# cruiseresearchgroup/ViLCo

Hardware: AMD Instinct MI355X
Metric: clips/sec (fwd+bwd) MQ transformer T=2304 C=2304 (higher is better)
Workload: dtype fp16 MFMA on 2-part splits of power-of-two scaled fp32 operands (22 significant bits, 3 MFMAs per product), fp32 accumulate: fp32-equivalent; weight-gradient products with contraction length >= 2048 use the leading fp16 parts only (11-bit operands, 1 MFMA; <= 3.5e-4 of the 3-MFMA gradients at this c; 1 GPU; MQ ViLCo backbone config P: T=2304 Cin=2304 D=1024 H=16 arch(2,2,5) XLNet layer text L=77x768 22 classes, train mode with the reference's dropout 0.1 / droppath 0.1 / XLNet dropout 0.1 (mq_vilco.yaml, xlnet_config_1024.json); clips_per_gpu=2, global_batch=2, parallelism=dp1

## Files before the change

vilco_amd/csrc/attn.hip:

```cpp
#include <type_traits>
#include "common.h"
#define VILCO_TU "attn"
#include "pack.h"

typedef __attribute__((ext_vector_type(4))) __bf16 bf16x4;
typedef __attribute__((ext_vector_type(4))) _Float16 f16x4;

namespace {

constexpr int ATT_THREADS = 256;

template <int W>
__device__ __forceinline__ int swzc(int row, int chunk) {
  if (W == 32) return chunk ^ ((4 - ((row >> 2) & 3)) & 3);
  if (W == 64) return chunk ^ ((row >> 1) & 7);
  if (W == 160) return (chunk & ~3) | ((chunk & 3) ^ ((4 - ((row >> 2) & 3)) & 3));
  return chunk ^ (row & 15);
}
template <int W>
__device__ __forceinline__ int toff(int row, int chunk) { return row * W + (swzc<W>(row, chunk) << 3); }

template <int NP>
__device__ __forceinline__ void split8(const float (&v)[8], bf16x8 (&part)[3]) {
#pragma unroll
// ... 349 lines not shown
      for (int q = 0; q < NP; ++q) pb[q] = frag<BKV>(myP + q * 16 * BKV, fb64, 0, ks);
#pragma unroll
      for (int di = 0; di < HDP / 16; ++di) {
        bf16x8 va[3];
#pragma unroll
        for (int q = 0; q < NP; ++q) va[q] = frag<BKV>(sVt + q * HDP * BKV, fb64, di * 16, ks);
        oacc[di] = mfma_parts<NP, F16>(va, pb, oacc[di]);
      }
    }
  }

  if (qi < a.Tq) {
    const float inv = (l_run > 0.f ? 1.f / l_run : 0.f) * (F16 ? P_INV * sc.iv : 1.f) * a.drop_inv_keep;
    float* og = a.o + ((long)b * a.Tq + qi) * ld + h * a.hd;
#pragma unroll
    for (int di = 0; di < HDP / 16; ++di) {
      const int d = di * 16 + (lane >> 4) * 4;
      if (d + 4 <= a.hd) {
        *reinterpret_cast<float4*>(og + d) = make_float4(oacc[di][0] * inv, oacc[di][1] * inv, oacc[di][2] * inv, oacc[di][3] * inv);
      } else {
#pragma unroll
        for (int r = 0; r < 4; ++r) if (d + r < a.hd) og[d + r] = oacc[di][r] * inv;
      }
    }
    if (a.lse && (lane >> 4) == 0) a.lse[(long)bh * a.Tq + qi] = m_run + logf(l_run);
  }
}

__device__ __forceinline__ f32x4 mfma3h(const bf16x8 (&a)[2], const bf16x8 (&b)[2], f32x4 c) {
  const f16x8 a0 = __builtin_bit_cast(f16x8, a[0]), a1 = __builtin_bit_cast(f16x8, a[1]);
  const f16x8 b0 = __builtin_bit_cast(f16x8, b[0]), b1 = __builtin_bit_cast(f16x8, b[1]);
  c = __builtin_amdgcn_mfma_f32_16x16x32_f16(a1, b0, c, 0, 0, 0);
  c = __builtin_amdgcn_mfma_f32_16x16x32_f16(a0, b1, c, 0, 0, 0);
  return __builtin_amdgcn_mfma_f32_16x16x32_f16(a0, b0, c, 0, 0, 0);
}

constexpr int F64_Q = 128;

__device__ __forceinline__ void block_amax_out(float m, float* out, float* smem_f) {
  m = wave_max(m);
  __syncthreads();
  if ((threadIdx.x & 63) == 0) smem_f[threadIdx.x >> 6] = m;
  __syncthreads();
  if (threadIdx.x == 0)
    out[(blockIdx.z * gridDim.y + blockIdx.y) * gridDim.x + blockIdx.x] = fmaxf(fmaxf(smem_f[0], smem_f[1]), fmaxf(smem_f[2], smem_f[3]));
}
constexpr int RS64 = 80;
constexpr int PL64 = 64 * RS64;

__device__ __forceinline__ bf16x8 tr_frag64(const __bf16* p) {
  typedef short s16x4 __attribute__((ext_vector_type(4)));
  const s16x4 lo = __builtin_amdgcn_ds_read_tr16_b64_v4i16((__attribute__((address_space(3))) s16x4*)(p));
  const s16x4 hi = __builtin_amdgcn_ds_read_tr16_b64_v4i16((__attribute__((address_space(3))) s16x4*)(p + 16 * RS64));
  return __builtin_bit_cast(bf16x8, __builtin_shufflevector(lo, hi, 0, 1, 2, 3, 4, 5, 6, 7));
}


#ifdef VILCO_LAB_ATTN
__device__ unsigned long long vilco_lab_attn_stamps[64 * 8];
#define ASTAMP(i)                                                                                             \
  do {                                                                                                         \
    if (stamp_on && stamp_t < 64) {                                                                            \
      const unsigned long long c_ = __builtin_amdgcn_s_memtime();                                              \
      asm volatile("s_waitcnt lgkmcnt(0)" ::: "memory");                                                       \
      if (lane == 0) vilco_lab_attn_stamps[stamp_t * 8 + (i)] = c_;                                            \
    }                                                                                                          \
  } while (0)
#else
#define ASTAMP(i) do {} while (0)
#endif

template <int NR>
__device__ __forceinline__ void xl_dma_rows(const float* bias, int ld, int Tq, int q_first, unsigned voff, unsigned lds0) {
#pragma unroll
  for (int r = 0; r < NR; ++r) {
    int qi = q_first + r;
    qi = qi < Tq ? qi : Tq - 1;
    const float* row = bias + ((long)qi * (ld - 1) + Tq);
    asm volatile("s_mov_b32 m0, %0\n\ts_nop 0\n\tglobal_load_lds_dword %1, %2" ::"s"(lds0 + (unsigned)r * 272u), "v"(voff), "s"(row) : "memory");
  }
}
__device__ __forceinline__ unsigned lds_addr_of(const void* p) {
  return (unsigned)(uintptr_t)(__attribute__((address_space(3))) const void*)p;
}

template <bool XL>
__global__ __launch_bounds__(ATT_THREADS, 2) void attn_fwd64_kernel(AttnArgs a) {
  if (a.drop_thresh) a.drop_seed = vilco_step_seed(a.drop_seed, a.seed_word);
  constexpr int HDP = 64, BKV = 64;
  extern __shared__ __attribute__((aligned(16))) unsigned char smem_raw[];
  __bf16* sK = reinterpret_cast<__bf16*>(smem_raw);
  __bf16* sV = sK + 2 * PL64;

  const int tid = threadIdx.x, lane = tid & 63, wave = tid >> 6;
  const int h = blockIdx.y, b = blockIdx.z;
  const int bh = b * a.H + h;
  const int q0 = blockIdx.x * F64_Q + wave * 32;
  const int len = a.mode == 2 ? a.Tk : a.kv_len[b];
  const int kend = XL ? a.Tk : (len < a.Tk ? len : a.Tk);
  const int ntiles = (kend + BKV - 1) / BKV;
  const AttnScales sc = *a.sc;
  const int bias_ld = a.Tq + a.Tk;
  const float* bias = XL ? a.bias + ((long)bh * a.Tq) * bias_ld : nullptr;
  constexpr int RSBF = 68;
  float* sBias = reinterpret_cast<float*>(sV + 2 * PL64) + wave * 32 * RSBF;
  const int q0s = __builtin_amdgcn_readfirstlane(q0);
  const unsigned sbias_lds = XL ? (unsigned)__builtin_amdgcn_readfirstlane((int)lds_addr_of(sBias)) : 0u;
  [[maybe_unused]] auto bias_dma = [&](int k0, int g) {
    const int j = k0 + lane;
    xl_dma_rows<16>(bias, bias_ld, a.Tq, q0s + 16 * g, 4u * (unsigned)(j < a.Tk ? j : a.Tk - 1), sbias_lds + (unsigned)g * 16u * 272u);
  };
  const float c2 = a.scale * sc.iq * sc.ik * 1.44269504088896340736f;
  const __bf16* kbase = a.kn.p + (long)bh * a.kn.batch_stride;
  const __bf16* vbase = a.vn.p + (long)bh * a.vn.batch_stride;
  const int g4 = lane >> 4;
  const int fbn = (lane & 15) * RS64 + g4 * 8;
  const int fbt = (4 * g4 + ((lane & 15) >> 2)) * RS64 + 4 * (lane & 3);

  QFrag<HDP, 2> qf[2];
#pragma unroll
  for (int g = 0; g < 2; ++g) load_qfrag<HDP, 2>(qf[g], a.qn, a.qn.p + (long)bh * a.qn.batch_stride, q0 + 16 * g, lane);

  f32x4 oacc[2][4];
#pragma unroll
  for (int g = 0; g < 2; ++g)
#pragma unroll
    for (int i = 0; i < 4; ++i) oacc[g][i] = f32x4{0.f, 0.f, 0.f, 0.f};
  float m_run[2] = {-INFINITY, -INFINITY}, l_run[2] = {0.f, 0.f};
  [[maybe_unused]] uint32_t rkey[2] = {0u, 0u};
  if constexpr (XL) {
    if (a.drop_thresh) { rkey[0] = drop_row(a, bh, q0 + (lane & 15)); rkey[1] = drop_row(a, bh, q0 + 16 + (lane & 15)); }
  }

  bf16x8 stK[2][2], stV[2][2];
  const int srow = tid >> 3, sc8 = tid & 7;
  auto gload = [&](int k0) {
#pragma unroll
    for (int i = 0; i < 2; ++i) {
      int kr = k0 + srow + 32 * i;
      kr = kr < a.kn.rows ? kr : a.kn.rows - 1;
#pragma unroll
      for (int q = 0; q < 2; ++q) {
        stK[q][i] = *reinterpret_cast<const bf16x8*>(kbase + q * a.kn.part_stride + (long)kr * HDP + sc8 * 8);
        stV[q][i] = *reinterpret_cast<const bf16x8*>(vbase + q * a.vn.part_stride + (long)kr * HDP + sc8 * 8);
      }
    }
  };
  auto lstore = [&]() {
#pragma unroll
    for (int i = 0; i < 2; ++i) {
      const int o = (srow + 32 * i) * RS64 + sc8 * 8;
#pragma unroll
      for (int q = 0; q < 2; ++q) {
        *reinterpret_cast<bf16x8*>(sK + q * PL64 + o) = stK[q][i];
        *reinterpret_cast<bf16x8*>(sV + q * PL64 + o) = stV[q][i];
      }
    }
  };

  typedef float f32x2 __attribute__((ext_vector_type(2)));
  typedef _Float16 f16x2 __attribute__((ext_vector_type(2)));
  typedef uint32_t u32x4 __attribute__((ext_vector_type(4)));
  const f32x2 c2v = {c2, c2};
#ifdef VILCO_LAB_ATTN
  const bool stamp_on = blockIdx.x == 0 && blockIdx.y == 0 && blockIdx.z == 0 && wave == 0;
#endif
// ... 68 lines not shown
      }
      float mx = fmaxf(fmaxf(s[g][0][0], s[g][0][1]), fmaxf(s[g][0][2], s[g][0][3]));
#pragma unroll
      for (int mi = 1; mi < 4; ++mi) mx = fmaxf(mx, fmaxf(fmaxf(s[g][mi][0], s[g][mi][1]), fmaxf(s[g][mi][2], s[g][mi][3])));
      mx = quad16_max(mx);
      const float m_new = fmaxf(m_run[g], mx);
      const bool dead = XL && m_new == -INFINITY;
      const float alpha = dead ? 1.f : __builtin_amdgcn_exp2f(m_run[g] - m_new);
      const float off = dead ? 0.f : 15.f - m_new;
      const f32x2 offv = {off, off};
      f32x2 psum = {0.f, 0.f};
#pragma unroll
      for (int ks = 0; ks < 2; ++ks) {
        u32x4 h0, h1;
#pragma unroll
        for (int e = 0; e < 8; e += 2) {
          const f32x2 sv = {s[g][2 * ks + (e >> 2)][e & 3], s[g][2 * ks + (e >> 2)][(e & 3) + 1]};
          const f32x2 arg = sv + offv;
          f32x2 p = {__builtin_amdgcn_exp2f(arg[0]), __builtin_amdgcn_exp2f(arg[1])};
          psum += p;
          if constexpr (XL) {
            if (a.drop_thresh) {
              const uint32_t jw = jw0 + (uint32_t)((2 * ks + (e >> 2)) * 16 + (e & 3)) * VILCO_ATTN_DROP_W;
              p[0] = vilco_attn_drop_keep_w(rkey[g], jw, a.drop_thresh) ? p[0] : 0.f;
              p[1] = vilco_attn_drop_keep_w(rkey[g], jw + VILCO_ATTN_DROP_W, a.drop_thresh) ? p[1] : 0.f;
            }
          }
          const f16x2 hp = {(_Float16)p[0], (_Float16)p[1]};
          const uint32_t hpu = __builtin_bit_cast(uint32_t, hp);
          uint32_t lo;
          asm("v_fma_mixlo_f16 %0, %1, -1.0, %2 op_sel_hi:[1,0,0]" : "=v"(lo) : "v"(hpu), "v"(p[0]));
          asm("v_fma_mixhi_f16 %0, %1, -1.0, %2 op_sel:[1,0,0] op_sel_hi:[1,0,0]" : "+v"(lo) : "v"(hpu), "v"(p[1]));
          h0[e >> 1] = hpu;
          h1[e >> 1] = lo;
        }
        pb[g][ks][0] = __builtin_bit_cast(bf16x8, h0);
        pb[g][ks][1] = __builtin_bit_cast(bf16x8, h1);
      }
      l_run[g] = l_run[g] * alpha + (psum[0] + psum[1]);
      m_run[g] = m_new;
      if (__any(alpha != 1.f)) {
#pragma unroll
        for (int i = 0; i < 4; ++i) { oacc[g][i][0] *= alpha; oacc[g][i][1] *= alpha; oacc[g][i][2] *= alpha; oacc[g][i][3] *= alpha; }
      }
      if constexpr (XL) {
        if (more) {
          asm volatile("s_waitcnt lgkmcnt(0)" ::: "memory");
          bias_dma(k0 + BKV, g);
        }
      }
    }
    ASTAMP(3);
    bf16x8 vf[2][2];
#pragma unroll
    for (int q = 0; q < 2; ++q) vf[0][q] = tr_frag64(sV + q * PL64 + fbt);
#pragma unroll
    for (int st = 0; st < 8; ++st) {
      const int ks = st >> 2, di = st & 3;
      if (st + 1 < 8) {
#pragma unroll
        for (int q = 0; q < 2; ++q) vf[(st + 1) & 1][q] = tr_frag64(sV + q * PL64 + fbt + ((st + 1) >> 2) * 32 * RS64 + ((st + 1) & 3) * 16);
      }
      const f16x8 v0h = __builtin_bit_cast(f16x8, vf[st & 1][0]), v1h = __builtin_bit_cast(f16x8, vf[st & 1][1]);
      const f16x8 a0 = __builtin_bit_cast(f16x8, pb[0][ks][0]), a1 = __builtin_bit_cast(f16x8, pb[0][ks][1]);
      const f16x8 b0 = __builtin_bit_cast(f16x8, pb[1][ks][0]), b1 = __builtin_bit_cast(f16x8, pb[1][ks][1]);
      f32x4 c0 = oacc[0][di], c1 = oacc[1][di];
      c0 = __builtin_amdgcn_mfma_f32_16x16x32_f16(v1h, a0, c0, 0, 0, 0);
      c1 = __builtin_amdgcn_mfma_f32_16x16x32_f16(v1h, b0, c1, 0, 0, 0);
      c0 = __builtin_amdgcn_mfma_f32_16x16x32_f16(v0h, a1, c0, 0, 0, 0);
      c1 = __builtin_amdgcn_mfma_f32_16x16x32_f16(v0h, b1, c1, 0, 0, 0);
      c0 = __builtin_amdgcn_mfma_f32_16x16x32_f16(v0h, a0, c0, 0, 0, 0);
      c1 = __builtin_amdgcn_mfma_f32_16x16x32_f16(v0h, b0, c1, 0, 0, 0);
      oacc[0][di] = c0; oacc[1][di] = c1;
    }
    ASTAMP(5);
  };

  if (ntiles > 0) gload(0);
  if constexpr (XL) { if (ntiles > 0) { bias_dma(0, 0); bias_dma(0, 1); } }
  const int nfull = (XL ? (len < a.Tk ? len : a.Tk) : kend) / BKV;
  for (int t = 0; t < nfull; ++t) tile(t, t + 1 < ntiles, std::false_type{});
  for (int t = nfull; t < ntiles; ++t) tile(t, t + 1 < ntiles, std::true_type{});

  typedef _Float16 h4o __attribute__((ext_vector_type(4)));
  const float so = a.op0 ? sc.sv * a.o_scale_mul : 0.f;
  float am = 0.f;
#pragma unroll
  for (int g = 0; g < 2; ++g) {
    float l = l_run[g];
    l = quad16_sum(l);
    const int qi = q0 + 16 * g + (lane & 15);
    if (qi < a.Tq) {
      const float inv = (l > 0.f ? 1.f / l : 0.f) * sc.iv * (XL ? a.drop_inv_keep : 1.f);
      float* og = a.o + ((long)b * a.Tq + qi) * a.C + h * HDP;
#pragma unroll
      for (int di = 0; di < 4; ++di) {
        const float4 v = make_float4(oacc[g][di][0] * inv, oacc[g][di][1] * inv, oacc[g][di][2] * inv, oacc[g][di][3] * inv);
        *reinterpret_cast<float4*>(og + di * 16 + g4 * 4) = v;
        am = fmaxf(fmaxf(am, fmaxf(fabsf(v.x), fabsf(v.y))), fmaxf(fabsf(v.z), fabsf(v.w)));
        if (a.op0) {
          const float xs[4] = {v.x * so, v.y * so, v.z * so, v.w * so};
          h4o h0, h1;
#pragma unroll
          for (int e = 0; e < 4; ++e) { h0[e] = (_Float16)xs[e]; h1[e] = (_Float16)(xs[e] - (float)h0[e]); }
          const long po = ((long)b * a.Tq + qi) * a.C + h * HDP + di * 16 + g4 * 4;
          *reinterpret_cast<h4o*>(a.op0 + po) = h0;
          *reinterpret_cast<h4o*>(a.op0 + a.o_plane_stride + po) = h1;
        }
      }
      if (a.lse && g4 == 0) a.lse[(long)bh * a.Tq + qi] = 0.69314718055994530942f * (m_run[g] + __builtin_amdgcn_logf(l) - 15.f);
    }
  }
  if (a.op0) {
    if ((blockIdx.x | blockIdx.y | blockIdx.z) == 0 && tid == 0) { a.o_inv_scale[0] = sc.iv / a.o_scale_mul; a.o_inv_scale[1] = so; }
    if (blockIdx.x == gridDim.x - 1 && b == a.B - 1) {
      const long rows = (long)a.B * a.Tq;
      const h4o hz = {(_Float16)0.f, (_Float16)0.f, (_Float16)0.f, (_Float16)0.f};
      for (long i = tid; i < (a.o_rows32 - rows) * 16; i += ATT_THREADS) {
        const long po = (rows + i / 16) * a.C + h * HDP + (i % 16) * 4;
        *reinterpret_cast<h4o*>(a.op0 + po) = hz;
        *reinterpret_cast<h4o*>(a.op0 + a.o_plane_stride + po) = hz;
      }
    }
  }
  if (a.am_o) block_amax_out(am, a.am_o, reinterpret_cast<float*>(smem_raw));
}

__global__ __launch_bounds__(ATT_THREADS, 2) void xl_scores64_kernel(AttnArgs a) {
  constexpr int HDP = 64;
  extern __shared__ __attribute__((aligned(16))) unsigned char smem_raw[];
  __bf16* sK = reinterpret_cast<__bf16*>(smem_raw);
  const int tid = threadIdx.x, lane = tid & 63, wave = tid >> 6;
  const int h = blockIdx.y, b = blockIdx.z;
  const int bh = b * a.H + h;
  const int T = a.Tq, P = 2 * a.Tq;
  const int Q0 = blockIdx.x * F64_Q, q0 = Q0 + wave * 32;
  const AttnScales sc = *a.sc;
  const float unscale = sc.iq * sc.ik;
  const __bf16* kbase = a.kn.p + (long)(a.mode ? bh : h) * a.kn.batch_stride;
  const int g4 = lane >> 4;
  const int fbn = (lane & 15) * RS64 + g4 * 8;

  QFrag<HDP, 2> qf[2];
#pragma unroll
  for (int g = 0; g < 2; ++g) load_qfrag<HDP, 2>(qf[g], a.qn, a.qn.p + (long)bh * a.qn.batch_stride, q0 + 16 * g, lane);

  bf16x8 stK[2][2];
  const int srow = tid >> 3, sc8 = tid & 7;
  auto gload = [&](int p0) {
#pragma unroll
    for (int i = 0; i < 2; ++i) {
      int kr = p0 + srow + 32 * i;
      kr = kr < a.kn.rows ? kr : a.kn.rows - 1;
#pragma unroll
      for (int q = 0; q < 2; ++q) stK[q][i] = *reinterpret_cast<const bf16x8*>(kbase + q * a.kn.part_stride + (long)kr * HDP + sc8 * 8);
    }
  };
  auto lstore = [&]() {
#pragma unroll
    for (int i = 0; i < 2; ++i) {
      const int o = (srow + 32 * i) * RS64 + sc8 * 8;
#pragma unroll
      for (int q = 0; q < 2; ++q) *reinterpret_cast<bf16x8*>(sK + q * PL64 + o) = stK[q][i];
    }
  };
  const int qlast = (Q0 + F64_Q - 1 < T ? Q0 + F64_Q - 1 : T - 1);
  const int t_lo = (T - qlast) / 64, t_hi = (P - Q0 + 63) / 64;
  float* orow[2];
  int irow[2];
#pragma unroll
  for (int g = 0; g < 2; ++g) {
    irow[g] = q0 + 16 * g + (lane & 15);
    orow[g] = a.o + ((long)bh * T + (irow[g] < T ? irow[g] : T - 1)) * P;
  }
  if (t_lo < t_hi) gload(t_lo * 64);
  for (int t = t_lo; t < t_hi; ++t) {
    const int p0 = t * 64;
    __syncthreads();
    lstore();
    __syncthreads();
    if (t + 1 < t_hi) gload(p0 + 64);
    if (p0 + 63 < T - (q0 + 31) || p0 >= P - q0) continue;
    f32x4 s[2][4];
    bf16x8 kf[2][2];
#pragma unroll
    for (int q = 0; q < 2; ++q) kf[0][q] = *reinterpret_cast<const bf16x8*>(sK + q * PL64 + fbn);
#pragma unroll
    for (int st = 0; st < 8; ++st) {
      const int mi = st >> 1, ks = st & 1;
      if (st + 1 < 8) {
#pragma unroll
        for (int q = 0; q < 2; ++q)
          kf[(st + 1) & 1][q] = *reinterpret_cast<const bf16x8*>(sK + q * PL64 + fbn + ((st + 1) >> 1) * 16 * RS64 + ((st + 1) & 1) * 32);
      }
      const f16x8 k0h = __builtin_bit_cast(f16x8, kf[st & 1][0]), k1h = __builtin_bit_cast(f16x8, kf[st & 1][1]);
      const f16x8 a0 = __builtin_bit_cast(f16x8, qf[0].f[ks][0]), a1 = __builtin_bit_cast(f16x8, qf[0].f[ks][1]);
      const f16x8 b0 = __builtin_bit_cast(f16x8, qf[1].f[ks][0]), b1 = __builtin_bit_cast(f16x8, qf[1].f[ks][1]);
      f32x4 c0 = ks ? s[0][mi] : f32x4{0.f, 0.f, 0.f, 0.f}, c1 = ks ? s[1][mi] : f32x4{0.f, 0.f, 0.f, 0.f};
      c0 = __builtin_amdgcn_mfma_f32_16x16x32_f16(k1h, a0, c0, 0, 0, 0);
      c1 = __builtin_amdgcn_mfma_f32_16x16x32_f16(k1h, b0, c1, 0, 0, 0);
      c0 = __builtin_amdgcn_mfma_f32_16x16x32_f16(k0h, a1, c0, 0, 0, 0);
      c1 = __builtin_amdgcn_mfma_f32_16x16x32_f16(k0h, b1, c1, 0, 0, 0);
      c0 = __builtin_amdgcn_mfma_f32_16x16x32_f16(k0h, a0, c0, 0, 0, 0);
      c1 = __builtin_amdgcn_mfma_f32_16x16x32_f16(k0h, b0, c1, 0, 0, 0);
      s[0][mi] = c0; s[1][mi] = c1;
    }
#pragma unroll
    for (int g = 0; g < 2; ++g) {
// ... 900 lines not shown
      const int off = toff<BQ>(ncol + (lane & 15), mq * 2 + (lane >> 5)) + ((lane >> 4) & 1) * 4;
#pragma unroll
      for (int q = 0; q < NP; ++q) {
        *reinterpret_cast<bf16x4*>(sPt + q * BKV * BQ + off) = pp[q];
        *reinterpret_cast<bf16x4*>(sdSt + q * BKV * BQ + off) = dd[q];
      }
    }
    __syncthreads();

    bf16x8 pb[3], sb[3];
#pragma unroll
    for (int q = 0; q < NP; ++q) {
      pb[q] = frag<BQ>(sPt + q * BKV * BQ, fb32, wave * 16, 0);
      sb[q] = frag<BQ>(sdSt + q * BKV * BQ, fb32, wave * 16, 0);
    }
#pragma unroll
    for (int di = 0; di < HDP / 16; ++di) {
      bf16x8 oa[3], qa[3];
#pragma unroll
      for (int q = 0; q < NP; ++q) {
        oa[q] = frag<BQ>(sdOt + q * HDP * BQ, fb32, di * 16, 0);
        qa[q] = frag<BQ>(sQt + q * HDP * BQ, fb32, di * 16, 0);
      }
      dvacc[di] = mfma_parts<NP, F16>(oa, pb, dvacc[di]);
      dkacc[di] = mfma_parts<NP, F16>(qa, sb, dkacc[di]);
    }
  }

  const int key = k0 + wave * 16 + (lane & 15);
  if (key < a.Tk) {
    float* gk = a.dk + ((long)b * a.Tk + key) * ld + h * a.hd;
    float* gv = a.dv + ((long)b * a.Tk + key) * ld + h * a.hd;
#pragma unroll
    for (int di = 0; di < HDP / 16; ++di) {
      const int d = di * 16 + (lane >> 4) * 4;
#pragma unroll
      for (int r = 0; r < 4; ++r) {
        if (d + r < a.hd) {
          gk[d + r] = dkacc[di][r] * (a.scale * ds_unscale * sc.iq);
          gv[d + r] = dvacc[di][r] * ((F16 ? P_INV * sc.ido : 1.f) * a.drop_inv_keep);
        }
      }
    }
  }
}

template <int HDP, int NP>
size_t fwd_lds() { return (size_t)NP * (64 * HDP + HDP * 64 + 4 * 16 * 64) * sizeof(__bf16); }
template <int HDP, int NP>
size_t dq_lds() { return (size_t)NP * (3 * 64 * HDP + 4 * 16 * 64) * sizeof(__bf16); }
template <int HDP, int NP>
size_t dkdv_lds() {
  return (size_t)NP * ((HDP > 128 ? 64 * HDP : 2 * 64 * HDP) + 4 * 32 * HDP + 2 * 64 * 32) * sizeof(__bf16);
}

template <typename K>
void set_lds(K kernel, size_t bytes) {
  hipFuncSetAttribute(reinterpret_cast<const void*>(kernel), hipFuncAttributeMaxDynamicSharedMemorySize, (int)bytes);
  (void)hipGetLastError();
}

bool fwd64_enabled();
inline bool fast64(const AttnArgs& a, int precision) {
  return precision == 3 && a.hd == 64 && !a.bias && !a.dbias && (a.mode == 0 || a.mode == 2) && !a.drop_thresh && fwd64_enabled();
}
bool xl64_enabled();
inline bool fast64_xl_fwd(const AttnArgs& a, int precision) {
  return precision == 3 && a.hd == 64 && a.bias && a.mode == 3 && a.Tq == a.Tk && fwd64_enabled() && xl64_enabled();
}
bool xl64_enabled() { static const bool on = [] { const char* e = getenv("VILCO_ATTN_XL_FAST"); return !(e && e[0] == '0'); }(); return on; }
bool fwd64_enabled() { static const bool on = [] { const char* e = getenv("VILCO_ATTN_FAST"); return !(e && e[0] == '0'); }(); return on; }

template <int HDP, int NP, bool F16 = false>
int launch_fwd(const AttnArgs& a, hipStream_t s) {
  if constexpr (HDP == 64 && NP == 2 && F16) {
    if (fast64(a, 3)) {
      size_t lds = 2 * 2 * PL64 * sizeof(__bf16);
#ifdef VILCO_LAB_ATTN
      if (const char* e = getenv("VILCO_LAB_ATTN_LDS")) {
        lds = (size_t)atoi(e);
        hipFuncSetAttribute(reinterpret_cast<const void*>(&attn_fwd64_kernel<false>), hipFuncAttributeMaxDynamicSharedMemorySize, (int)lds);
      }
#endif
      hipLaunchKernelGGL(attn_fwd64_kernel<false>, dim3((a.Tq + F64_Q - 1) / F64_Q, a.H, a.B), dim3(ATT_THREADS), lds, s, a);
      return vilco_launch_status();
    }
    if (fast64_xl_fwd(a, 3)) {
      const size_t lds = 2 * 2 * PL64 * sizeof(__bf16) + 4 * 32 * 68 * sizeof(float);
      static const bool oncexl = [] { set_lds(&attn_fwd64_kernel<true>, 2 * 2 * PL64 * sizeof(__bf16) + 4 * 32 * 68 * sizeof(float)); return true; }();
      (void)oncexl;
      hipLaunchKernelGGL(attn_fwd64_kernel<true>, dim3((a.Tq + F64_Q - 1) / F64_Q, a.H, a.B), dim3(ATT_THREADS), lds, s, a);
      return vilco_launch_status();
    }
  }
  static const bool once = [] {
    set_lds(&attn_fwd_kernel<HDP, NP, F16, false>, fwd_lds<HDP, NP>());
    set_lds(&attn_fwd_kernel<HDP, NP, F16, true>, fwd_lds<HDP, NP>());
    return true;
  }();
  (void)once;
  dim3 grid((a.Tq + 63) / 64, a.H, a.B);
  const size_t lds = fwd_lds<HDP, NP>();
  if (a.drop_thresh) hipLaunchKernelGGL((attn_fwd_kernel<HDP, NP, F16, true>), grid, dim3(ATT_THREADS), lds, s, a);
  else hipLaunchKernelGGL((attn_fwd_kernel<HDP, NP, F16, false>), grid, dim3(ATT_THREADS), lds, s, a);
  return vilco_launch_status();
}

struct ForkCtx { hipStream_t s2; hipEvent_t e0, e1; };

inline ForkCtx* attn_fork(hipStream_t s) {
  static const bool enabled = [] { const char* e = getenv("VILCO_ATTN_FORK"); return e && e[0] == '1'; }();
  if (!enabled) return nullptr;
  hipStreamCaptureStatus st = hipStreamCaptureStatusNone;
  if (hipStreamIsCapturing(s, &st) != hipSuccess) return nullptr;
  static ForkCtx ctx;
  static int state = 0;
  if (st != hipStreamCaptureStatusActive) {
    if (state == 0)
      state = (hipStreamCreateWithFlags(&ctx.s2, hipStreamNonBlocking) == hipSuccess &&
               hipEventCreateWithFlags(&ctx.e0, hipEventDisableTiming) == hipSuccess &&
               hipEventCreateWithFlags(&ctx.e1, hipEventDisableTiming) == hipSuccess) ? 1 : -1;
    return nullptr;
  }
  return state == 1 ? &ctx : nullptr;
}

template <int HDP, int NP, bool F16 = false>
int launch_bwd(const AttnArgs& a, hipStream_t s) {
  static const bool once = [] {
    set_lds(&attn_bwd_dq_kernel<HDP, NP, F16, false>, dq_lds<HDP, NP>());
    set_lds(&attn_bwd_dq_kernel<HDP, NP, F16, true>, dq_lds<HDP, NP>());
    set_lds(&attn_bwd_dkdv_kernel<HDP, NP, F16, false, false>, dkdv_lds<HDP, NP>());
    set_lds(&attn_bwd_dkdv_kernel<HDP, NP, F16, true, false>, dkdv_lds<HDP, NP>());
    set_lds(&attn_bwd_dkdv_kernel<HDP, NP, F16, false, true>, dkdv_lds<HDP, NP>());
    set_lds(&attn_bwd_dkdv_kernel<HDP, NP, F16, true, true>, dkdv_lds<HDP, NP>());
    return true;
  }();
  (void)once;
  dim3 gq((a.Tq + 63) / 64, a.H, a.B), gk((a.Tk + 63) / 64, a.H, a.B);
  const size_t lq = dq_lds<HDP, NP>(), lk = dkdv_lds<HDP, NP>();
  (void)attn_fork(s);
  bool fast = false;
  if constexpr (HDP == 64 && NP == 2 && F16)
    fast = fast64(a, 3);
  if (fast) {
    if constexpr (HDP == 64 && NP == 2 && F16) {
      constexpr size_t l64 = 2 * 2 * PL64 * sizeof(__bf16);
      const dim3 gq64((a.Tq + F64_Q - 1) / F64_Q, a.H, a.B);
      ForkCtx* f = (long)gq64.x * gq64.y * gq64.z > 512 ? attn_fork(s) : nullptr;
      if (f) {
        hipLaunchKernelGGL(attn_delta64_kernel, dim3((a.Tq + 63) / 64, a.H, a.B), dim3(256), 0, s, a);
        hipEventRecord(f->e0, s);
        hipStreamWaitEvent(f->s2, f->e0, 0);
        hipLaunchKernelGGL(attn_bwd_dq64_kernel<false>, gq64, dim3(ATT_THREADS), l64, s, a);
        hipLaunchKernelGGL(attn_bwd_dkdv64_kernel<false>, gk, dim3(ATT_THREADS), l64, f->s2, a);
        hipEventRecord(f->e1, f->s2);
        hipStreamWaitEvent(s, f->e1, 0);
        return vilco_launch_status();
      }
      hipLaunchKernelGGL(attn_bwd_dq64_kernel<false>, gq64, dim3(ATT_THREADS), l64, s, a);
      hipLaunchKernelGGL(attn_bwd_dkdv64_kernel<false>, gk, dim3(ATT_THREADS), l64, s, a);
      return vilco_launch_status();
    }
  }
  bool xl_dq = false;
  if constexpr (HDP == 64 && NP == 2 && F16) xl_dq = fast64_xl_fwd(a, 3) && (a.dbias != nullptr || a.dsp != nullptr);
// ... 371 lines not shown
```

Measured before the change: 98.43 clips/s.

## Add software-pipelined non-XL fwd64 attention kernel overlapping QK with softmax/PV

Adds a new forward attention kernel for head dim 64 that computes the QK^T scores of the next KV tile while doing softmax and PV on the current one. K and V are double-buffered separately in LDS and prefetched from global two or three tiles ahead. The shared epilogue moves into a helper function. The aim is to hide softmax and global-load latency behind MFMA work, at the cost of twice the LDS and more live registers, which may lower occupancy. It is used for the non-XL path when Tk > 128.

```diff
diff --git a/vilco_amd/csrc/attn.hip b/vilco_amd/csrc/attn.hip
--- a/vilco_amd/csrc/attn.hip
+++ b/vilco_amd/csrc/attn.hip
@@ -455,6 +455,56 @@
 }
 __device__ __forceinline__ unsigned lds_addr_of(const void* p) {
   return (unsigned)(uintptr_t)(__attribute__((address_space(3))) const void*)p;
+}
+
+template <bool XL>
+__device__ __forceinline__ void fwd64_finish(const AttnArgs& a, const AttnScales& sc, const f32x4 (&oacc)[2][4], const float (&l_run)[2],
+                                             const float (&m_run)[2], int q0, unsigned char* smem_raw) {
+  constexpr int HDP = 64;
+  const int tid = threadIdx.x, lane = tid & 63, g4 = lane >> 4;
+  const int h = blockIdx.y, b = blockIdx.z, bh = b * a.H + h;
+  typedef _Float16 h4o __attribute__((ext_vector_type(4)));
+  const float so = a.op0 ? sc.sv * a.o_scale_mul : 0.f;
+  float am = 0.f;
+#pragma unroll
+  for (int g = 0; g < 2; ++g) {
+    float l = l_run[g];
+    l = quad16_sum(l);
+    const int qi = q0 + 16 * g + (lane & 15);
+    if (qi < a.Tq) {
+      const float inv = (l > 0.f ? 1.f / l : 0.f) * sc.iv * (XL ? a.drop_inv_keep : 1.f);
+      float* og = a.o + ((long)b * a.Tq + qi) * a.C + h * HDP;
+#pragma unroll
+      for (int di = 0; di < 4; ++di) {
+        const float4 v = make_float4(oacc[g][di][0] * inv, oacc[g][di][1] * inv, oacc[g][di][2] * inv, oacc[g][di][3] * inv);
+        *reinterpret_cast<float4*>(og + di * 16 + g4 * 4) = v;
+        am = fmaxf(fmaxf(am, fmaxf(fabsf(v.x), fabsf(v.y))), fmaxf(fabsf(v.z), fabsf(v.w)));
+        if (a.op0) {
+          const float xs[4] = {v.x * so, v.y * so, v.z * so, v.w * so};
+          h4o h0, h1;
+#pragma unroll
+          for (int e = 0; e < 4; ++e) { h0[e] = (_Float16)xs[e]; h1[e] = (_Float16)(xs[e] - (float)h0[e]); }
+          const long po = ((long)b * a.Tq + qi) * a.C + h * HDP + di * 16 + g4 * 4;
+          *reinterpret_cast<h4o*>(a.op0 + po) = h0;
+          *reinterpret_cast<h4o*>(a.op0 + a.o_plane_stride + po) = h1;
+        }
+      }
+      if (a.lse && g4 == 0) a.lse[(long)bh * a.Tq + qi] = 0.69314718055994530942f * (m_run[g] + __builtin_amdgcn_logf(l) - 15.f);
+    }
+  }
+  if (a.op0) {
+    if ((blockIdx.x | blockIdx.y | blockIdx.z) == 0 && tid == 0) { a.o_inv_scale[0] = sc.iv / a.o_scale_mul; a.o_inv_scale[1] = so; }
+    if (blockIdx.x == gridDim.x - 1 && b == a.B - 1) {
+      const long rows = (long)a.B * a.Tq;
+      const h4o hz = {(_Float16)0.f, (_Float16)0.f, (_Float16)0.f, (_Float16)0.f};
+      for (long i = tid; i < (a.o_rows32 - rows) * 16; i += ATT_THREADS) {
+        const long po = (rows + i / 16) * a.C + h * HDP + (i % 16) * 4;
+        *reinterpret_cast<h4o*>(a.op0 + po) = hz;
+        *reinterpret_cast<h4o*>(a.op0 + a.o_plane_stride + po) = hz;
+      }
+    }
+  }
+  if (a.am_o) block_amax_out(am, a.am_o, reinterpret_cast<float*>(smem_raw));
 }
 
 template <bool XL>
@@ -689,48 +739,219 @@
   for (int t = 0; t < nfull; ++t) tile(t, t + 1 < ntiles, std::false_type{});
   for (int t = nfull; t < ntiles; ++t) tile(t, t + 1 < ntiles, std::true_type{});
 
-  typedef _Float16 h4o __attribute__((ext_vector_type(4)));
-  const float so = a.op0 ? sc.sv * a.o_scale_mul : 0.f;
-  float am = 0.f;
-#pragma unroll
-  for (int g = 0; g < 2; ++g) {
-    float l = l_run[g];
-    l = quad16_sum(l);
-    const int qi = q0 + 16 * g + (lane & 15);
-    if (qi < a.Tq) {
-      const float inv = (l > 0.f ? 1.f / l : 0.f) * sc.iv * (XL ? a.drop_inv_keep : 1.f);
-      float* og = a.o + ((long)b * a.Tq + qi) * a.C + h * HDP;
-#pragma unroll
-      for (int di = 0; di < 4; ++di) {
-        const float4 v = make_float4(oacc[g][di][0] * inv, oacc[g][di][1] * inv, oacc[g][di][2] * inv, oacc[g][di][3] * inv);
-        *reinterpret_cast<float4*>(og + di * 16 + g4 * 4) = v;
-        am = fmaxf(fmaxf(am, fmaxf(fabsf(v.x), fabsf(v.y))), fmaxf(fabsf(v.z), fabsf(v.w)));
-        if (a.op0) {
-          const float xs[4] = {v.x * so, v.y * so, v.z * so, v.w * so};
-          h4o h0, h1;
-#pragma unroll
-          for (int e = 0; e < 4; ++e) { h0[e] = (_Float16)xs[e]; h1[e] = (_Float16)(xs[e] - (float)h0[e]); }
-          const long po = ((long)b * a.Tq + qi) * a.C + h * HDP + di * 16 + g4 * 4;
-          *reinterpret_cast<h4o*>(a.op0 + po) = h0;
-          *reinterpret_cast<h4o*>(a.op0 + a.o_plane_stride + po) = h1;
+  fwd64_finish<XL>(a, sc, oacc, l_run, m_run, q0, smem_raw);
+}
+
+__global__ __launch_bounds__(ATT_THREADS, 2) void attn_fwd64p_kernel(AttnArgs a) {
+  constexpr int HDP = 64, BKV = 64;
+  extern __shared__ __attribute__((aligned(16))) unsigned char smem_raw[];
+  __bf16* sK = reinterpret_cast<__bf16*>(smem_raw);
+  __bf16* sV = sK + 4 * PL64;
+
+  const int tid = threadIdx.x, lane = tid & 63, wave = tid >> 6;
+  const int h = blockIdx.y, b = blockIdx.z;
+  const int bh = b * a.H + h;
+  const int q0 = blockIdx.x * F64_Q + wave * 32;
+  const int len = a.mode == 2 ? a.Tk : a.kv_len[b];
+  const int kend = len < a.Tk ? len : a.Tk;
+  const int ntiles = (kend + BKV - 1) / BKV;
+  const AttnScales sc = *a.sc;
+  const float c2 = a.scale * sc.iq * sc.ik * 1.44269504088896340736f;
+  const __bf16* kbase = a.kn.p + (long)bh * a.kn.batch_stride;
+  const __bf16* vbase = a.vn.p + (long)bh * a.vn.batch_stride;
+  const int g4 = lane >> 4;
+  const int fbn = (lane & 15) * RS64 + g4 * 8;
+  const int fbt = (4 * g4 + ((lane & 15) >> 2)) * RS64 + 4 * (lane & 3);
+
+  QFrag<HDP, 2> qf[2];
+#pragma unroll
+  for (int g = 0; g < 2; ++g) load_qfrag<HDP, 2>(qf[g], a.qn, a.qn.p + (long)bh * a.qn.batch_stride, q0 + 16 * g, lane);
+
+  f32x4 oacc[2][4];
+#pragma unroll
+  for (int g = 0; g < 2; ++g)
+#pragma unroll
+    for (int i = 0; i < 4; ++i) oacc[g][i] = f32x4{0.f, 0.f, 0.f, 0.f};
+  float m_run[2] = {-INFINITY, -INFINITY}, l_run[2] = {0.f, 0.f};
+
+  bf16x8 stK[2][2], stV[2][2];
+  const int srow = tid >> 3, sc8 = tid & 7;
+  auto gload1 = [&](bf16x8 (&st)[2][2], const __bf16* base, const Planes& pl, int k0) {
+#pragma unroll
+    for (int i = 0; i < 2; ++i) {
+      int kr = k0 + srow + 32 * i;
+      kr = kr < pl.rows ? kr : pl.rows - 1;
+#pragma unroll
+      for (int q = 0; q < 2; ++q) st[q][i] = *reinterpret_cast<const bf16x8*>(base + q * pl.part_stride + (long)kr * HDP + sc8 * 8);
+    }
+  };
+  auto lstore1 = [&](__bf16* dst, const bf16x8 (&st)[2][2]) {
+#pragma unroll
+    for (int i = 0; i < 2; ++i)
+#pragma unroll
+      for (int q = 0; q < 2; ++q) *reinterpret_cast<bf16x8*>(dst + q * PL64 + (srow + 32 * i) * RS64 + sc8 * 8) = st[q][i];
+  };
+
+  typedef _Float16 f16x2 __attribute__((ext_vector_type(2)));
+  typedef uint32_t u32x4 __attribute__((ext_vector_type(4)));
+#ifdef VILCO_LAB_ATTN
+  const bool stamp_on = blockIdx.x == 0 && blockIdx.y == 0 && blockIdx.z == 0 && wave == 0;
+  int stamp_t = 0;
+#endif
+
+  auto s_mma = [&](const __bf16* ks, f32x4 (&s)[2][4]) {
+    bf16x8 kf[2][2];
+#pragma unroll
+    for (int q = 0; q < 2; ++q) kf[0][q] = *reinterpret_cast<const bf16x8*>(ks + q * PL64 + fbn);
+#pragma unroll
+    for (int st = 0; st < 8; ++st) {
+      const int mi = st >> 1, ks2 = st & 1;
+      if (st + 1 < 8) {
+#pragma unroll
+        for (int q = 0; q < 2; ++q)
+          kf[(st + 1) & 1][q] = *reinterpret_cast<const bf16x8*>(ks + q * PL64 + fbn + ((st + 1) >> 1) * 16 * RS64 + ((st + 1) & 1) * 32);
+      }
+      const f16x8 k0h = __builtin_bit_cast(f16x8, kf[st & 1][0]), k1h = __builtin_bit_cast(f16x8, kf[st & 1][1]);
+      const f16x8 a0 = __builtin_bit_cast(f16x8, qf[0].f[ks2][0]), a1 = __builtin_bit_cast(f16x8, qf[0].f[ks2][1]);
+      const f16x8 b0 = __builtin_bit_cast(f16x8, qf[1].f[ks2][0]), b1 = __builtin_bit_cast(f16x8, qf[1].f[ks2][1]);
+      f32x4 c0 = ks2 ? s[0][mi] : f32x4{0.f, 0.f, 0.f, 0.f}, c1 = ks2 ? s[1][mi] : f32x4{0.f, 0.f, 0.f, 0.f};
+      c0 = __builtin_amdgcn_mfma_f32_16x16x32_f16(k1h, a0, c0, 0, 0, 0);
+      c1 = __builtin_amdgcn_mfma_f32_16x16x32_f16(k1h, b0, c1, 0, 0, 0);
+      c0 = __builtin_amdgcn_mfma_f32_16x16x32_f16(k0h, a1, c0, 0, 0, 0);
+      c1 = __builtin_amdgcn_mfma_f32_16x16x32_f16(k0h, b1, c1, 0, 0, 0);
+      c0 = __builtin_amdgcn_mfma_f32_16x16x32_f16(k0h, a0, c0, 0, 0, 0);
+      c1 = __builtin_amdgcn_mfma_f32_16x16x32_f16(k0h, b0, c1, 0, 0, 0);
+      s[0][mi] = c0; s[1][mi] = c1;
+    }
+  };
+  auto softmax = [&](f32x4 (&s)[2][4], bf16x8 (&pb)[2][2][2], float (&alpha)[2]) {
+#pragma unroll
+    for (int g = 0; g < 2; ++g) {
+#pragma unroll
+      for (int mi = 0; mi < 4; ++mi)
+#pragma unroll
+        for (int r = 0; r < 4; ++r) s[g][mi][r] *= c2;
+      float mx = fmaxf(fmaxf(s[g][0][0], s[g][0][1]), fmaxf(s[g][0][2], s[g][0][3]));
+#pragma unroll
+      for (int mi = 1; mi < 4; ++mi) mx = fmaxf(mx, fmaxf(fmaxf(s[g][mi][0], s[g][mi][1]), fmaxf(s[g][mi][2], s[g][mi][3])));
+      mx = quad16_max(mx);
+      const float m_new = fmaxf(m_run[g], mx);
+      alpha[g] = __builtin_amdgcn_exp2f(m_run[g] - m_new);
+      const float off = 15.f - m_new;
+      float psum0 = 0.f, psum1 = 0.f;
+#pragma unroll
+      for (int ks = 0; ks < 2; ++ks) {
+        u32x4 h0, h1;
+#pragma unroll
+        for (int e = 0; e < 8; e += 2) {
+          const float p0 = __builtin_amdgcn_exp2f(s[g][2 * ks + (e >> 2)][e & 3] + off);
+          const float p1 = __builtin_amdgcn_exp2f(s[g][2 * ks + (e >> 2)][(e & 3) + 1] + off);
+          psum0 += p0;
+          psum1 += p1;
+          const f16x2 hp = {(_Float16)p0, (_Float16)p1};
+          const uint32_t hpu = __builtin_bit_cast(uint32_t, hp);
+          uint32_t lo;
+          asm("v_fma_mixlo_f16 %0, %1, -1.0, %2 op_sel_hi:[1,0,0]" : "=v"(lo) : "v"(hpu), "v"(p0));
+          asm("v_fma_mixhi_f16 %0, %1, -1.0, %2 op_sel:[1,0,0] op_sel_hi:[1,0,0]" : "+v"(lo) : "v"(hpu), "v"(p1));
+          h0[e >> 1] = hpu;
+          h1[e >> 1] = lo;
         }
-      }
-      if (a.lse && g4 == 0) a.lse[(long)bh * a.Tq + qi] = 0.69314718055994530942f * (m_run[g] + __builtin_amdgcn_logf(l) - 15.f);
-    }
-  }
-  if (a.op0) {
-    if ((blockIdx.x | blockIdx.y | blockIdx.z) == 0 && tid == 0) { a.o_inv_scale[0] = sc.iv / a.o_scale_mul; a.o_inv_scale[1] = so; }
-    if (blockIdx.x == gridDim.x - 1 && b == a.B - 1) {
-      const long rows = (long)a.B * a.Tq;
-      const h4o hz = {(_Float16)0.f, (_Float16)0.f, (_Float16)0.f, (_Float16)0.f};
-      for (long i = tid; i < (a.o_rows32 - rows) * 16; i += ATT_THREADS) {
-        const long po = (rows + i / 16) * a.C + h * HDP + (i % 16) * 4;
-        *reinterpret_cast<h4o*>(a.op0 + po) = hz;
-        *reinterpret_cast<h4o*>(a.op0 + a.o_plane_stride + po) = hz;
-      }
-    }
-  }
-  if (a.am_o) block_amax_out(am, a.am_o, reinterpret_cast<float*>(smem_raw));
+        pb[g][ks][0] = __builtin_bit_cast(bf16x8, h0);
+        pb[g][ks][1] = __builtin_bit_cast(bf16x8, h1);
+      }
+      l_run[g] = l_run[g] * alpha[g] + (psum0 + psum1);
+      m_run[g] = m_new;
+    }
+  };
+  auto pv_mma = [&](const __bf16* vs, const bf16x8 (&pb)[2][2][2], const float (&alpha)[2]) {
+    if (__any(alpha[0] != 1.f || alpha[1] != 1.f)) {
+#pragma unroll
+      for (int g = 0; g < 2; ++g)
+#pragma unroll
+        for (int i = 0; i < 4; ++i) { oacc[g][i][0] *= alpha[g]; oacc[g][i][1] *= alpha[g]; oacc[g][i][2] *= alpha[g]; oacc[g][i][3] *= alpha[g]; }
+    }
+    bf16x8 vf[2][2];
+#pragma unroll
+    for (int q = 0; q < 2; ++q) vf[0][q] = tr_frag64(vs + q * PL64 + fbt);
+#pragma unroll
+    for (int st = 0; st < 8; ++st) {
+      const int ks = st >> 2, di = st & 3;
+      if (st + 1 < 8) {
+#pragma unroll
+        for (int q = 0; q < 2; ++q) vf[(st + 1) & 1][q] = tr_frag64(vs + q * PL64 + fbt + ((st + 1) >> 2) * 32 * RS64 + ((st + 1) & 3) * 16);
+      }
+      const f16x8 v0h = __builtin_bit_cast(f16x8, vf[st & 1][0]), v1h = __builtin_bit_cast(f16x8, vf[st & 1][1]);
+      const f16x8 a0 = __builtin_bit_cast(f16x8, pb[0][ks][0]), a1 = __builtin_bit_cast(f16x8, pb[0][ks][1]);
+      const f16x8 b0 = __builtin_bit_cast(f16x8, pb[1][ks][0]), b1 = __builtin_bit_cast(f16x8, pb[1][ks][1]);
+      f32x4 c0 = oacc[0][di], c1 = oacc[1][di];
+      c0 = __builtin_amdgcn_mfma_f32_16x16x32_f16(v1h, a0, c0, 0, 0, 0);
+      c1 = __builtin_amdgcn_mfma_f32_16x16x32_f16(v1h, b0, c1, 0, 0, 0);
+      c0 = __builtin_amdgcn_mfma_f32_16x16x32_f16(v0h, a1, c0, 0, 0, 0);
+      c1 = __builtin_amdgcn_mfma_f32_16x16x32_f16(v0h, b1, c1, 0, 0, 0);
+      c0 = __builtin_amdgcn_mfma_f32_16x16x32_f16(v0h, a0, c0, 0, 0, 0);
+      c1 = __builtin_amdgcn_mfma_f32_16x16x32_f16(v0h, b0, c1, 0, 0, 0);
+      oacc[0][di] = c0; oacc[1][di] = c1;
+    }
+  };
+  auto step = [&](int t, f32x4 (&sc_)[2][4], f32x4 (&sn)[2][4]) {
+#ifdef VILCO_LAB_ATTN
+    stamp_t = t;
+#endif
+    ASTAMP(0);
+    __syncthreads();
+    lstore1(sK + (t & 1) * 2 * PL64, stK);
+    lstore1(sV + ((t + 1) & 1) * 2 * PL64, stV);
+    ASTAMP(1);
+    if (t + 3 < ntiles) gload1(stK, kbase, a.kn, (t + 3) * BKV);
+    if (t + 2 < ntiles) gload1(stV, vbase, a.vn, (t + 2) * BKV);
+    ASTAMP(2);
+    bf16x8 pb[2][2][2];
+    float alpha[2];
+    s_mma(sK + ((t + 1) & 1) * 2 * PL64, sn);
+    softmax(sc_, pb, alpha);
+    ASTAMP(3);
+    pv_mma(sV + (t & 1) * 2 * PL64, pb, alpha);
+    ASTAMP(5);
+  };
+  auto last = [&](int t, f32x4 (&sc_)[2][4]) {
+#ifdef VILCO_LAB_ATTN
+    stamp_t = t;
+#endif
+    ASTAMP(0);
+    __syncthreads();
+    ASTAMP(1);
+    ASTAMP(2);
+#pragma unroll
+    for (int mi = 0; mi < 4; ++mi)
+#pragma unroll
+      for (int r = 0; r < 4; ++r)
+        if (t * BKV + mi * 16 + g4 * 4 + r >= kend) { sc_[0][mi][r] = -INFINITY; sc_[1][mi][r] = -INFINITY; }
+    bf16x8 pb[2][2][2];
+    float alpha[2];
+    softmax(sc_, pb, alpha);
+    ASTAMP(3);
+    pv_mma(sV + (t & 1) * 2 * PL64, pb, alpha);
+    ASTAMP(5);
+  };
+
+  if (ntiles > 0) {
+    f32x4 s0[2][4], s1[2][4];
+    gload1(stK, kbase, a.kn, 0);
+    gload1(stV, vbase, a.vn, 0);
+    lstore1(sK, stK);
+    lstore1(sV, stV);
+    if (ntiles > 1) gload1(stK, kbase, a.kn, BKV);
+    __syncthreads();
+    s_mma(sK, s0);
+    lstore1(sK + 2 * PL64, stK);
+    if (ntiles > 2) gload1(stK, kbase, a.kn, 2 * BKV);
+    if (ntiles > 1) gload1(stV, vbase, a.vn, BKV);
+    int t = 0;
+    for (; t + 2 < ntiles; t += 2) { step(t, s0, s1); step(t + 1, s1, s0); }
+    if (t + 1 < ntiles) { step(t, s0, s1); last(t + 1, s1); }
+    else last(t, s0);
+  }
+  fwd64_finish<false>(a, sc, oacc, l_run, m_run, q0, smem_raw);
 }
 
 __global__ __launch_bounds__(ATT_THREADS, 2) void xl_scores64_kernel(AttnArgs a) {
@@ -1797,6 +2018,13 @@
         hipFuncSetAttribute(reinterpret_cast<const void*>(&attn_fwd64_kernel<false>), hipFuncAttributeMaxDynamicSharedMemorySize, (int)lds);
       }
 #endif
+      if (a.Tk > 128) {
+        constexpr size_t ldsp = 2 * 2 * 2 * PL64 * sizeof(__bf16);
+        static const bool oncep = [] { set_lds(&attn_fwd64p_kernel, ldsp); return true; }();
+        (void)oncep;
+        hipLaunchKernelGGL(attn_fwd64p_kernel, dim3((a.Tq + F64_Q - 1) / F64_Q, a.H, a.B), dim3(ATT_THREADS), ldsp, s, a);
+        return vilco_launch_status();
+      }
       hipLaunchKernelGGL(attn_fwd64_kernel<false>, dim3((a.Tq + F64_Q - 1) / F64_Q, a.H, a.B), dim3(ATT_THREADS), lds, s, a);
       return vilco_launch_status();
     }
```

Result: no change. 98.31 clips/s, median of 2 (-0.1%).
